# megvii-research/CVPR2023-UniDistill

Measured on AMD Instinct MI355X. Metric: distill-train samples/sec (nuScenes frame); bev_pool+voxelize HBM GB/s, higher is better.
Workload: dtype f32; 1 GPU; camera_exp_distill_lidar: student+teacher distillation step, 6 cams 256x704, 30000-pt cloud, 40 GT boxes, fwd+bwd+AdamW; batch_per_gpu=4, global_batch=4, parallelism=dp1, layout=channels-last dense convs, executor=eager+DDP, strict_no_library_fallthrough=True, wgrad_stream=on, ranks=1, dist_backend=none (single process)

## Files before the change

cvpr2023-unidistill_amd/csrc/conv2d_f32_wino4.hip:

```cpp
#include "ud_common.h"
#include "ud_prof.h"
#include <cstdlib>
#include <type_traits>
#include <utility>
#include <algorithm>

#ifndef UD_W4_ABL
#define UD_W4_ABL 0
#endif

namespace {

typedef float f32x4 __attribute__((ext_vector_type(4)));
typedef float f32x2 __attribute__((ext_vector_type(2)));

constexpr int kT = 32, kTN = 64, kKC = 4, kFQ = 9;
constexpr int kUBytes = kFQ * kTN * kKC * 16;
constexpr int kVBytes = kFQ * kT * kKC * 16;
constexpr int kPBytes = 21504;
constexpr int kP0 = 0, kU0 = 2 * kPBytes, kV0 = kU0 + kUBytes, kV1 = kV0 + kVBytes, kU1 = kV1 + kVBytes;
constexpr int kDump = kU1 + kUBytes;
constexpr int kSmem = kDump + 1024;
constexpr int kStageA = 0, kStageB = kDump - 65536;
static_assert(kStageB >= kV0 && kV1 == kV0 + kVBytes && 65536 <= kV0 + kVBytes, "LDS map");

struct W4Geom {
  int B, H, W, Cin, Cout, bx, by;
  unsigned u_bytes;
  int n_dp, n_units, sk_len;
  float* partial;
};
struct W4Ep {
  const float* bias;
  const float* scale;
  const float* shift;
  const float* residual;
  int relu;
  float* stats;
};

__device__ __forceinline__ void dma16(__amdgpu_buffer_rsrc_t rsrc, unsigned voff, unsigned soff, unsigned lds_wave_base) {
  __builtin_amdgcn_raw_ptr_buffer_load_lds(rsrc, (__attribute__((address_space(3))) void*)(size_t)lds_wave_base, 16, voff, soff, 0, 0);
}
constexpr unsigned kOob = 0xFFF00000u;

__device__ __forceinline__ f32x2 pk_fma(f32x2 a, f32x2 b, f32x2 c) {
  f32x2 d;
  asm("v_pk_fma_f32 %0, %1, %2, %3" : "=v"(d) : "s"(a), "v"(b), "v"(c));
  return d;
}
// ... 75 lines not shown
    u[4] = (1.f / 24.f) * a - (1.f / 12.f) * b + (1.f / 6.f) * cc2;
    u[5] = cc2;
#pragma unroll
    for (int j = 0; j < 6; ++j) {
      const int f = w4_f(r, j);
      out[(f >> 2) * (64 * 16) + (f & 3)] = u[j];
    }
  }
}

template <int N>
struct IC {
  static constexpr int value = N;
};
template <typename F, int... Is>
__device__ __forceinline__ void static_for_impl(F&& f, std::integer_sequence<int, Is...>) {
  (f(IC<Is>{}), ...);
}
template <int N, typename F>
__device__ __forceinline__ void static_for(F&& f) {
  static_for_impl(std::forward<F>(f), std::make_integer_sequence<int, N>{});
}

template <int TWB, int THB>
struct W4Tail {
  const W4Geom& gm;
  const W4Ep& ep;
  int b, ty0, tx0, n0, tid, c4, n;
  float4 bv, scv, shv, s1, s2;
  __device__ W4Tail(const W4Geom& gm_, const W4Ep& ep_, int b_, int ty0_, int tx0_, int n0_, int tid_)
      : gm(gm_), ep(ep_), b(b_), ty0(ty0_), tx0(tx0_), n0(n0_), tid(tid_) {
    c4 = (tid & 15) * 4, n = n0 + c4;
    bv = make_float4(0.f, 0.f, 0.f, 0.f), scv = make_float4(1.f, 1.f, 1.f, 1.f), shv = bv, s1 = bv, s2 = bv;
    if (ep.bias && n < gm.Cout) bv = *reinterpret_cast<const float4*>(ep.bias + n);
    if (ep.scale && n < gm.Cout) {
      scv = *reinterpret_cast<const float4*>(ep.scale + n);
      shv = *reinterpret_cast<const float4*>(ep.shift + n);
    }
  }
  __device__ __forceinline__ void store(float* __restrict__ y, int pass, int row, float4 v) {
    static_assert((TWB & (TWB - 1)) == 0, "tile-block width: a power of two (shift / mask below)");
    const int tl = row >> 4, p = row & 15;
    const int slot = 16 * (tl >> 3) + 4 * ((tl >> 1) & 3) + 2 * pass + (tl & 1);
    const int sy = slot / TWB, sx = slot & (TWB - 1);
    const int gy = 4 * (ty0 + sy) + (p >> 2), gx = 4 * (tx0 + sx) + (p & 3);
    if (slot >= TWB * THB || gy >= gm.H || gx >= gm.W || n >= gm.Cout) return;
    if (ep.bias) { v.x += bv.x; v.y += bv.y; v.z += bv.z; v.w += bv.w; }
    if (ep.scale) {
      v.x = v.x * scv.x + shv.x; v.y = v.y * scv.y + shv.y; v.z = v.z * scv.z + shv.z; v.w = v.w * scv.w + shv.w;
    }
    const size_t off = ((size_t)(b * gm.H + gy) * gm.W + gx) * gm.Cout + n;
    if (ep.residual) {
      const float4 h = *reinterpret_cast<const float4*>(ep.residual + off);
      v.x += h.x; v.y += h.y; v.z += h.z; v.w += h.w;
    }
    if (ep.relu) {
      v.x = fmaxf(v.x, 0.f); v.y = fmaxf(v.y, 0.f); v.z = fmaxf(v.z, 0.f); v.w = fmaxf(v.w, 0.f);
    }
    *reinterpret_cast<float4*>(y + off) = v;
    if (ep.stats) {
      s1.x += v.x; s1.y += v.y; s1.z += v.z; s1.w += v.w;
      s2.x += v.x * v.x; s2.y += v.y * v.y; s2.z += v.z * v.z; s2.w += v.w * v.w;
    }
  }
  __device__ void reduce_stats(float* red, int blk_lin) {
    const int grp = tid >> 4;
    const float a4[4] = {s1.x, s1.y, s1.z, s1.w}, q4[4] = {s2.x, s2.y, s2.z, s2.w};
#pragma unroll
    for (int e = 0; e < 4; ++e) {
      red[(grp * 64 + c4 + e) * 2] = a4[e];
      red[(grp * 64 + c4 + e) * 2 + 1] = q4[e];
    }
    __syncthreads();
    if (tid < 64 && n0 + tid < gm.Cout) {
      double ad = 0.0, qd = 0.0;
      for (int k = 0; k < 32; ++k) {
        ad += (double)red[(k * 64 + tid) * 2];
        qd += (double)red[(k * 64 + tid) * 2 + 1];
      }
      ep.stats[((size_t)blk_lin * gm.Cout + n0 + tid) * 2] = (float)ad;
      ep.stats[((size_t)blk_lin * gm.Cout + n0 + tid) * 2 + 1] = (float)qd;
    }
  }
};

__device__ constexpr int kStepOps[9] = {3, 3, 3, 3, 0, 0, 0, 4, 0};
__host__ __device__ constexpr int w4_wait(int fq) {
  return (fq > 0 ? kStepOps[fq - 1] : 0) + 2 + kStepOps[fq];
}

template <int TWB, int THB>
__global__ __launch_bounds__(512) void k_conv3x3_wino4_f32(const float* __restrict__ x, const float* __restrict__ U,
                                                           float* __restrict__ y, W4Geom gm, W4Ep ep) {
  constexpr int PW = 4 * TWB + 2, PH = 4 * THB + 2;
  constexpr int RP = (TWB == 16) ? PW : (PW | 1);
  constexpr int RB = 2 * RP * 16;
  constexpr int PP = PH * 2 * RP, kPInstr = (PP + 63) / 64;
  static_assert(TWB * THB <= kT && kPInstr * 1024 <= kPBytes && kPInstr <= 24, "tile block");
  constexpr int O0 = 0, O1 = TWB + 1, O2 = 2 * TWB + 2, O3 = 3 * TWB + 2;
  static_assert((O3 + 0) * 4 <= 255 && (O1 + 1) * 4 <= 255, "ds_read2 offsets");
  extern __shared__ __attribute__((aligned(16))) char smem[];
  const unsigned sbase = (unsigned)(size_t)smem;
  const int tid = threadIdx.x, lane = tid & 63;
  const int wave = __builtin_amdgcn_readfirstlane(tid >> 6);
  const int g = lane >> 4, li = lane & 15;
  const int wq = wave & 3, wh = wave >> 2;
  const int nblocks = gm.B * gm.bx * gm.by;
  const int nchunks = gm.Cin / kKC;
  const __amdgpu_buffer_rsrc_t rx = __builtin_amdgcn_make_buffer_rsrc((void*)x, 0, (int)((unsigned)gm.B * gm.H * gm.W * gm.Cin * 4u), 0x00020000);
  const __amdgpu_buffer_rsrc_t ru = __builtin_amdgcn_make_buffer_rsrc((void*)U, 0, (int)gm.u_bytes, 0x00020000);

  int unit, cbi, blk_lin, b, ty0, tx0, n0;
  unsigned po[3];
  unsigned uo;
  unsigned pair_off;
  int nst;
  auto setup = [&](int unit_, int c0, int c1) {
    unit = unit_;
    nst = c1 - c0;
    cbi = unit / nblocks;
    const int ru_ = unit - cbi * nblocks;
    int blk;
    {
      const int base = nblocks >> 3, extra = nblocks & 7, k = ru_ & 7;
      blk = k * base + min(k, extra) + (ru_ >> 3);
    }
    blk_lin = blk;
    b = blk / (gm.bx * gm.by);
    blk -= b * gm.bx * gm.by;
    ty0 = (blk / gm.bx) * THB, tx0 = (blk % gm.bx) * TWB;
    n0 = cbi * kTN;
#pragma unroll
    for (int i = 0; i < 3; ++i) {
      const int pi = wave + 8 * i;
      const int qq = pi * 64 + lane;
      const int qy = qq / (2 * RP), qr = qq - qy * (2 * RP);
      const int qh = qr >= RP ? 1 : 0, qs = qr - qh * RP;
      const int qx = qs < O1 ? 4 * qs : qs < O2 ? 4 * (qs - O1) + 1 : qs < O3 ? 4 * (qs - O2) + 2 : 4 * (qs - O3) + 3;
      const int gy = 4 * ty0 + qy - 1, gx = 4 * tx0 + qx - 1;
      const bool ok = qq < PP && qs < PW && gy >= 0 && gy < gm.H && gx >= 0 && gx < gm.W && !(UD_W4_ABL & (2 | 128));
      po[i] = ok ? (unsigned)(((b * gm.H + gy) * gm.W + gx) * gm.Cin + qh * 4) * 4u : kOob;
    }
    uo = (unsigned)(cbi * nchunks + c0) * (unsigned)kUBytes + wave * 1024;
    pair_off = c0 * 16;
  };
  auto patch_piece = [&](int i, int buf) {
    const int pi = wave + 8 * i;
    dma16(rx, po[i], pair_off, pi < kPInstr ? sbase + kP0 + buf * kPBytes + pi * 1024 : sbase + kDump);
  };
  const unsigned lane16 = lane * 16;
  auto stage_u = [&](int buf) {
    const unsigned ub = sbase + (buf ? kU1 : kU0) + wave * 1024;
#pragma unroll
    for (int i = 0; i < 5; ++i)
      if (i < 4 || wave < 4) dma16(ru, lane16, uo + i * 8192, ub + i * 8192);
  };

  const int grp = wave >> 1;
  const int ttile = (wave & 1) * 16 + (lane & 15), tc = lane >> 4;
  const int ttc = min(ttile, TWB * THB - 1);
  const int tyl = ttc / TWB, txl = ttc - tyl * TWB;
  const unsigned tprow = sbase + kP0 + (4 * tyl) * RB + txl * 16 + tc * 4;
  const int rows4 = grp == 0 ? 0x4420 : grp == 1 ? 0x5531 : 0x1324;
  const unsigned ro1 = (rows4 & 15) * RB, ro2 = ((rows4 >> 4) & 15) * RB, ro3 = ((rows4 >> 8) & 15) * RB, ro4 = ((rows4 >> 12) & 15) * RB;
  const float ca1 = grp < 2 ? 4.f : 1.f, ca2 = grp < 2 ? -5.f : grp == 2 ? -4.f : -1.f;
  const float cb3 = grp == 0 ? 1.f : grp == 1 ? -1.f : grp == 2 ? 1.f : 2.f, cb4 = grp < 2 ? 0.f : grp == 2 ? -4.f : -2.f;
  const unsigned tvbase = sbase + kV0 + (wave & 1) * 1024 + lane * 16;
  const unsigned tdump = sbase + kDump + lane * 16;
  const int q0 = grp < 2 ? 0 : grp == 2 ? 3 : 6;
  const unsigned wA = grp == 1 ? tdump : tvbase + q0 * (kT * kKC * 16);
  const unsigned wB = grp == 1 ? tdump : tvbase + (q0 + 1) * (kT * kKC * 16);
  const unsigned wC = grp == 0 ? tdump : tvbase + (q0 + 1) * (kT * kKC * 16) + 8;
  const unsigned wD = grp == 0 ? tdump : tvbase + (q0 + 2) * (kT * kKC * 16);
  const unsigned vdelta01 = (grp == 1 ? 0 : kVBytes), vdelta23 = (grp == 0 ? 0 : kVBytes);

#define W4_ROWREAD(D, RO)                                                                                               \
  do {                                                                                                                  \
    const unsigned a_ = tprow + (RO);                                                                                   \
    asm volatile("ds_read2_b32 %0, %1 offset0:%2 offset1:%3" : "=v"(D[0]) : "v"(a_), "n"(O0 * 4), "n"(O1 * 4));               \
    asm volatile("ds_read2_b32 %0, %1 offset0:%2 offset1:%3" : "=v"(D[1]) : "v"(a_), "n"(O2 * 4), "n"(O3 * 4));               \
    asm volatile("ds_read2_b32 %0, %1 offset0:%2 offset1:%3" : "=v"(D[2]) : "v"(a_), "n"((O0 + 1) * 4), "n"((O1 + 1) * 4));   \
  } while (0)

  auto row_pass = [](const f32x2 (&w)[3], f32x2 (&v)[3]) {
    const f32x2 c4 = {4.f, 4.f}, c5 = {-5.f, -5.f}, c41 = {-4.f, -1.f}, c12 = {1.f, 2.f}, cn12 = {-1.f, -2.f};
// ... 150 lines not shown
  if (!next_piece()) return;
  setup(p_unit, p_c0, p_c1);
  first_stages();
#pragma unroll 1
  for (;;) {
    asm volatile("s_waitcnt vmcnt(0)" ::: "memory");
    __syncthreads();
    transform_first();
#pragma unroll
    for (int f = 0; f < 36; ++f) acc[f] = (f32x4){0.f, 0.f, 0.f, 0.f};
    asm volatile("s_waitcnt lgkmcnt(0)" ::: "memory");
    __syncthreads();
    asm volatile("ds_read_b128 %0, %1" : "=v"(qa[0]) : "v"(fa));
    asm volatile("ds_read_b128 %0, %1" : "=v"(qb[0]) : "v"(fb0 + kU0));
#pragma unroll 1
    for (int chunk = 0; chunk < nst; chunk += 2) {
      stage(IC<0>{}, chunk);
      stage(IC<1>{}, chunk + 1);
    }
    asm volatile("s_waitcnt vmcnt(0) lgkmcnt(0)" : "+v"(qa[0]), "+v"(qb[0]), "+v"(qa[1]), "+v"(qb[1])::"memory");
    __syncthreads();
    const int e_b = b, e_ty0 = ty0, e_tx0 = tx0, e_n0 = n0, e_blk = blk_lin, e_slot = p_slot;
    const bool more = next_piece();
    W4Tail<TWB, THB> tail(gm, ep, e_b, e_ty0, e_tx0, e_n0, tid);
#pragma unroll
    for (int pass = (UD_W4_ABL & 4) ? 1 : 0; pass < 2; ++pass) {
      float* Os = reinterpret_cast<float*>(smem + (pass ? kStageB : kStageA));
      {
        auto m2 = [&](int i, int j) { return (f32x2){acc[w4_f(i, j)][2 * pass], acc[w4_f(i, j)][2 * pass + 1]}; };
        const f32x2 c2 = {2.f, 2.f}, c4 = {4.f, 4.f}, c8 = {8.f, 8.f};
        f32x2 t[4][6];
#pragma unroll
        for (int j = 0; j < 6; ++j) {
          const f32x2 m1 = m2(1, j), mm2 = m2(2, j), m3 = m2(3, j), m4 = m2(4, j);
          const f32x2 sa = m1 + mm2, da = m1 - mm2, sb = m3 + m4, db = m3 - m4;
          t[0][j] = m2(0, j) + sa + sb;
          t[1][j] = __builtin_elementwise_fma(c2, db, da);
          t[2][j] = __builtin_elementwise_fma(c4, sb, sa);
          t[3][j] = __builtin_elementwise_fma(c8, db, da) + m2(5, j);
        }
        const unsigned o = sbase + (pass ? kStageB : kStageA) + ((wh * 8 + g * 2) * 16 * 64 + (16 * (wq ^ g) + li)) * 4;
#pragma unroll
        for (int a = 0; a < 4; ++a) {
          const f32x2 sa = t[a][1] + t[a][2], da = t[a][1] - t[a][2], sb = t[a][3] + t[a][4], db = t[a][3] - t[a][4];
          const f32x2 y0 = t[a][0] + sa + sb, y1 = __builtin_elementwise_fma(c2, db, da), y2 = __builtin_elementwise_fma(c4, sb, sa),
                      y3 = __builtin_elementwise_fma(c8, db, da) + t[a][5];
          asm volatile("ds_write2st64_b32 %0, %1, %2 offset0:%3 offset1:%4" ::"v"(o), "v"(y0.x), "v"(y0.y), "n"(a * 4 + 0), "n"(a * 4 + 16) : "memory");
// ... 14 lines not shown
#pragma unroll
        for (int k = 0; k < 8; ++k) {
          const int row = (tid >> 4) + 32 * k;
          *reinterpret_cast<float4*>(dst + row * 64 + tail.c4) =
              *reinterpret_cast<const float4*>(Os + row * 64 + (tail.c4 ^ (16 * ((row >> 5) & 3))));
        }
      }
      if (pass == 0) {
        __syncthreads();
        if (more) {
          setup(p_unit, p_c0, p_c1);
          first_stages();
        }
      }
    }
    if (ep.stats && e_slot < 0) {
      __syncthreads();
      tail.reduce_stats(reinterpret_cast<float*>(smem + kStageB), e_blk);
    }
    if (!more) break;
  }
}

template <int TWB, int THB>
__global__ __launch_bounds__(512) void k_wino4_fixup(float* __restrict__ y, W4Geom gm, W4Ep ep) {
  __shared__ float red[32 * 64 * 2];
  const int tid = threadIdx.x;
  const int nblocks = gm.B * gm.bx * gm.by, nchunks = gm.Cin / kKC;
  const int u = gm.n_dp + (blockIdx.x >> 1), pass = blockIdx.x & 1;
  const int base = gm.n_dp * nchunks;
  const int a = u * nchunks - base, e = a + nchunks - 1;
  const int j0 = a / gm.sk_len, j1 = e / gm.sk_len;
  if (j0 == j1) return;
  const int cbi = u / nblocks, ru = u - cbi * nblocks;
  int blk;
  {
    const int bs = nblocks >> 3, extra = nblocks & 7, k = ru & 7;
    blk = k * bs + min(k, extra) + (ru >> 3);
  }
  const int blk_lin = blk;
  const int b = blk / (gm.bx * gm.by);
  blk -= b * gm.bx * gm.by;
  W4Tail<TWB, THB> tail(gm, ep, b, (blk / gm.bx) * THB, (blk % gm.bx) * TWB, cbi * kTN, tid);
  float4 v[8];
#pragma unroll
  for (int k = 0; k < 8; ++k) v[k] = make_float4(0.f, 0.f, 0.f, 0.f);
#pragma unroll 1
  for (int j = j0; j <= j1; ++j) {
    const int first_unit = (base + j * gm.sk_len) / nchunks;
    const int slot = 2 * j + (first_unit == u ? 0 : 1);
    const float* src = gm.partial + ((size_t)slot * 512 + pass * 256 + (tid >> 4)) * 64 + tail.c4;
#pragma unroll
    for (int k = 0; k < 8; ++k) {
      const float4 p = ud_ldg_stream(src + (size_t)k * 32 * 64);
      v[k].x += p.x; v[k].y += p.y; v[k].z += p.z; v[k].w += p.w;
    }
  }
#pragma unroll
  for (int k = 0; k < 8; ++k) tail.store(y, pass, (tid >> 4) + 32 * k, v[k]);
  if (ep.stats) {
    tail.reduce_stats(red, nblocks + 2 * (u - gm.n_dp) + pass);
    if (pass == 0 && tid < 64 && tail.n0 + tid < gm.Cout)
      ep.stats[((size_t)blk_lin * gm.Cout + tail.n0 + tid) * 2] = ep.stats[((size_t)blk_lin * gm.Cout + tail.n0 + tid) * 2 + 1] = 0.f;
  }
}

#undef W4_ROWREAD
#undef W4_COL

struct W4Plan {
  int twb, thb, bx, by;
};
W4Plan w4_plan(int H, int W) {
  static const int shapes[][2] = {{8, 4}, {4, 8}, {16, 2}};
  static const int force = getenv("UD_WINO4_SHAPE") ? atoi(getenv("UD_WINO4_SHAPE")) : -1;
  const int TX = (W + 3) / 4, TY = (H + 3) / 4;
  W4Plan best{};
  long long cost = -1;
  for (int i = 0; i < 3; ++i) {
    if (force >= 0 && i != force) continue;
    const int bx = ud_div_up(TX, shapes[i][0]), by = ud_div_up(TY, shapes[i][1]);
    const long long cst = (long long)bx * by;
    if (cost < 0 || cst < cost) cost = cst, best = W4Plan{shapes[i][0], shapes[i][1], bx, by};
  }
  return best;
}

}

namespace {
std::atomic<int> g_sk_mode{-1};
constexpr int kGrid = 256;
struct W4Sched {
  int grid, n_dp, sk_len;
};
W4Sched w4_schedule(long long units, int nchunks, bool have_ws) {
  static const int env_mode = getenv("UD_WINO4_SK") ? atoi(getenv("UD_WINO4_SK")) : 2;
  const int forced = g_sk_mode.load(std::memory_order_relaxed);
  const int mode = forced >= 0 ? forced : env_mode;
  static const int persist = getenv("UD_WINO4_GRID") ? atoi(getenv("UD_WINO4_GRID")) : kGrid;
  const int G = (int)std::min<long long>(units, persist);
  const int r = (int)(units % G);
  W4Sched sc{G, (int)units, 0};
  if (r == 0 || !have_ws || !mode || (nchunks < 64 && mode < 2)) return sc;
  int len = (int)(((long long)r * nchunks + G - 1) / G);
  len += len & 1;
  if (len + 16 >= (nchunks + 8) * 9 / 10) return sc;
  sc.n_dp = (int)(units - r), sc.sk_len = len;
  return sc;
}
}

extern "C" size_t ud_conv3x3_wino4_f32_weight_bytes(int Cin, int Cout) {
  if (Cin <= 0 || Cout <= 0) return 0;
  return (size_t)ud_div_up(Cout, 64) * ud_div_up(Cin, 4) * kUBytes;
}

extern "C" int ud_conv3x3_wino4_f32_blocks(int H, int W) {
  if (H <= 0 || W <= 0) return 0;
  const W4Plan p = w4_plan(H, W);
  return p.bx * p.by;
}

extern "C" size_t ud_conv3x3_wino4_bnstats_bytes(int B, int H, int W, int Cout) {
  if (B <= 0 || H <= 0 || W <= 0 || Cout <= 0) return 0;
  const W4Plan p = w4_plan(H, W);
  return ((size_t)B * p.bx * p.by + 2 * kGrid) * Cout * 2 * sizeof(float);
}

extern "C" int ud_conv3x3_wino4_f32_weights(const float* w, int64_t s_n, int64_t s_c, int64_t s_y, int64_t s_x, int N, int C,
                                            int flip, float* U, ud_stream_t stream_) {
  if (!w || !U || N <= 0 || C <= 0) return UD_ERR_INVALID_ARG;
  hipStream_t stream = (hipStream_t)stream_;
  UdProfScope prof("conv2d.k_wino4_weights", stream);
  const long long total = (long long)ud_div_up(N, 64) * ud_div_up(C, 4) * 256;
  k_wino4_weights<<<(unsigned)((total + 255) / 256), 256, 0, stream>>>(w, s_n, s_c, s_y, s_x, N, C, flip, U, total);
  UD_LAUNCH_CHECK();
  return UD_OK;
}

extern "C" void ud_conv3x3_wino4_stream_k(int mode) { g_sk_mode.store(mode, std::memory_order_relaxed); }

extern "C" size_t ud_conv3x3_wino4_f32_workspace_bytes(int B, int H, int W, int Cin, int Cout) {
  (void)B; (void)H; (void)W; (void)Cin; (void)Cout;
  return (size_t)2 * kGrid * 512 * 64 * sizeof(float);
}

extern "C" int ud_conv3x3_wino4_nhwc_f32(const float* x, const float* U, float* y, int B, int H, int W, int Cin, int Cout,
                                         const float* bias, const float* scale, const float* shift, const float* residual,
                                         int flags, float* partial, size_t partial_bytes, int* slices, void* workspace,
                                         size_t workspace_bytes, ud_stream_t stream_) {
  if (!x || !U || !y || B <= 0 || H <= 0 || W <= 0 || Cin <= 0 || Cout <= 0) return UD_ERR_INVALID_ARG;
  if ((scale == nullptr) != (shift == nullptr)) return UD_ERR_INVALID_ARG;
  if (Cin % (2 * kKC) != 0 || Cout % 4 != 0) return UD_ERR_UNSUPPORTED;
  hipStream_t stream = (hipStream_t)stream_;
  const W4Plan p = w4_plan(H, W);
  const int nblocks = B * p.bx * p.by;
  const long long units = (long long)nblocks * ud_div_up(Cout, kTN);
  if (units > 0x7fffffffll || (long long)B * H * W * Cin * 4 >= (long long)kOob ||
      ud_conv3x3_wino4_f32_weight_bytes(Cin, Cout) >= (size_t)kOob)
    return UD_ERR_UNSUPPORTED;
  const bool have_ws = workspace && workspace_bytes >= ud_conv3x3_wino4_f32_workspace_bytes(B, H, W, Cin, Cout);
  const W4Sched sc = w4_schedule(units, Cin / kKC, have_ws);
  W4Geom gm{B, H, W, Cin, Cout, p.bx, p.by, (unsigned)ud_conv3x3_wino4_f32_weight_bytes(Cin, Cout), sc.n_dp, (int)units,
            sc.sk_len > 0 ? sc.sk_len : 2, (float*)workspace};
  W4Ep ep{bias, scale, shift, residual, flags & 1, partial};
  if (partial) {
    const size_t rows = (size_t)nblocks + 2 * (size_t)(units - sc.n_dp);
    if (!slices || partial_bytes < rows * Cout * 2 * sizeof(float)) return UD_ERR_WORKSPACE;
    *slices = (int)rows;
    if (rows > (size_t)nblocks)
      ud_zero_f32_async(partial + (size_t)nblocks * Cout * 2, (rows - nblocks) * (size_t)Cout * 2, stream);
  }
  static UdDeviceOnce attr_set;
  if (const unsigned long long attr_set_bit = attr_set.pending()) {
#define UD_W4_ATTR(A, Bq) \
  UD_HIP_TRY(hipFuncSetAttribute((const void*)k_conv3x3_wino4_f32<A, Bq>, hipFuncAttributeMaxDynamicSharedMemorySize, kSmem))
    UD_W4_ATTR(8, 4); UD_W4_ATTR(4, 8); UD_W4_ATTR(16, 2);
#undef UD_W4_ATTR
    attr_set.mark(attr_set_bit);
  }
  UdProfScope prof("conv2d.k_conv3x3_wino4_f32", stream);
  const dim3 grid((unsigned)sc.grid);
  const int n_sk = (int)units - sc.n_dp;
#define UD_W4_LAUNCH(A, Bq)                                                                    \
  do {                                                                                         \
    k_conv3x3_wino4_f32<A, Bq><<<grid, 512, kSmem, stream>>>(x, U, y, gm, ep);                 \
    if (n_sk > 0) k_wino4_fixup<A, Bq><<<2 * n_sk, 512, 0, stream>>>(y, gm, ep);               \
  } while (0)
  if (p.twb == 8) UD_W4_LAUNCH(8, 4);
  else if (p.twb == 4) UD_W4_LAUNCH(4, 8);
  else UD_W4_LAUNCH(16, 2);
#undef UD_W4_LAUNCH
  UD_LAUNCH_CHECK();
  return UD_OK;
}
```

cvpr2023-unidistill_amd/unidistill_amd/_lib.py:

```python
import ctypes
import os

import torch

_HERE = os.path.dirname(os.path.abspath(__file__))
LIB_PATH = os.path.join(_HERE, "_lib", "libunidistill_hip.so")
_cdll = None

c_void_p, c_int, c_size_t, c_uint, c_i64, c_float = (
    ctypes.c_void_p, ctypes.c_int, ctypes.c_size_t, ctypes.c_uint, ctypes.c_int64, ctypes.c_float)

_SIGS = {
    "ud_version": (ctypes.c_char_p, []),
    "ud_abi_version": (c_int, []),
    "ud_error_string": (ctypes.c_char_p, [c_int]),
    "ud_prof_enable": (None, [c_int]),
    "ud_prof_read": (c_int, [ctypes.c_char_p, ctypes.POINTER(ctypes.c_double), ctypes.POINTER(c_int), c_int]),
    "ud_bench_stream": (c_int, [c_void_p, c_void_p, c_size_t, c_int, c_void_p]),
    "ud_bev_pool_workspace_bytes": (c_size_t, [c_int] * 6),
    "ud_bev_pool_fwd": (c_int, [c_void_p] * 4 + [c_int] * 6 + [c_uint, c_void_p, c_size_t, c_void_p]),
    "ud_bev_pool_bwd_workspace_bytes": (c_size_t, [c_int] * 4 + [c_i64]),
    "ud_bev_pool_bwd": (c_int, [c_void_p] + [c_i64] * 4 + [c_void_p, c_void_p] + [c_int] * 5
                        + [c_void_p, c_size_t, c_void_p]),
    "ud_lss_prepare_mats": (c_int, [c_void_p] * 6 + [c_int, c_int, c_void_p, c_void_p]),
# ... 95 lines not shown
                            + [c_size_t, c_void_p]),
    "ud_lidar_prep_compact": (c_int, [c_void_p, c_i64, c_int, c_void_p, c_void_p, c_int, c_int] + [c_void_p] * 6
                              + [c_i64, c_int, c_void_p, c_i64, c_void_p, c_size_t, c_void_p]),
    "ud_jpeg_parse": (c_int, [c_void_p, c_i64, c_void_p]),
    "ud_jpeg_plan": (c_size_t, [c_void_p, c_int]),
    "ud_jpeg_decode": (c_int, [c_void_p, c_i64, c_void_p, c_void_p, c_int, c_void_p, c_i64, c_void_p, c_void_p,
                               c_void_p, c_size_t, c_void_p]),
    "ud_nus_pred_to_global": (c_int, [c_void_p, c_i64, c_int] + [c_void_p] * 3 + [c_int, c_void_p, c_int]
                              + [c_void_p] * 7),
    "ud_nus_eval_workspace_bytes": (c_size_t, [c_i64, c_int]),
    "ud_nus_eval": (c_int, [c_void_p, c_void_p, c_int, c_i64, c_void_p, c_size_t, c_void_p]),
    "ud_stem_pack_weights": (c_int, [c_void_p] + [c_i64] * 4 + [c_void_p]),
    "ud_stem_conv7x7_bn_relu": (c_int, [c_void_p] + [c_i64] * 4 + [c_int] * 3 + [c_void_p] * 4 + [c_int, c_void_p]),
    "ud_maxpool3x3s2_nhwc": (c_int, [c_void_p] * 2 + [c_int] * 5 + [c_void_p]),
    "ud_conv1x1_wgrad_workspace_bytes": (c_size_t, [c_i64, c_int, c_int]),
    "ud_conv3x3_wgrad_f32_workspace_bytes": (c_size_t, [c_int] * 5),
    "ud_conv3x3_wgrad_nhwc_f32": (c_int, [c_void_p] * 3 + [c_int] * 5 + [c_void_p, c_size_t, c_void_p]),
    "ud_conv1x1_wgrad_f32_workspace_bytes": (c_size_t, [c_i64, c_int, c_int]),
    "ud_conv1x1_wgrad_mapped_nhwc_f32": (c_int, [c_void_p] * 3 + [c_i64, c_int, c_int] + [c_void_p] * 2
                                         + [c_void_p, c_size_t, c_void_p]),
    "ud_conv3x3_wino4_f32_weight_bytes": (c_size_t, [c_int, c_int]),
    "ud_conv3x3_wino4_bnstats_bytes": (c_size_t, [c_int] * 4),
    "ud_conv3x3_wino4_f32_blocks": (c_int, [c_int, c_int]),
    "ud_conv3x3_wino4_f32_weights": (c_int, [c_void_p] + [c_i64] * 4 + [c_int] * 3 + [c_void_p, c_void_p]),
    "ud_conv3x3_wino4_f32_workspace_bytes": (c_size_t, [c_int] * 5),
    "ud_conv3x3_wino4_stream_k": (None, [c_int]),
    "ud_conv3x3_wino4_nhwc_f32": (c_int, [c_void_p] * 3 + [c_int] * 5 + [c_void_p] * 4 + [c_int, c_void_p, c_size_t,
                                                                                              c_void_p, c_void_p, c_size_t, c_void_p]),
    "ud_conv3x3_wino_f32_weight_bytes": (c_size_t, [c_int, c_int]),
    "ud_conv3x3_wino_bnstats_bytes": (c_size_t, [c_int] * 4),
    "ud_conv3x3_wino4_wgrad_f32_workspace_bytes": (c_size_t, [c_int] * 5),
    "ud_conv3x3_wino4_wgrad_nhwc_f32": (c_int, [c_void_p] * 3 + [c_int] * 5 + [c_void_p, c_size_t, c_void_p]),
    "ud_conv3x3_wino_wgrad_f32_workspace_bytes": (c_size_t, [c_int] * 5),
    "ud_conv3x3_wino_wgrad_nhwc_f32": (c_int, [c_void_p] * 3 + [c_int] * 5 + [c_void_p, c_size_t, c_void_p]),
    "ud_conv3x3_wino_f32_blocks": (c_int, [c_int, c_int]),
    "ud_conv3x3_wino_f32_weights": (c_int, [c_void_p] + [c_i64] * 4 + [c_int] * 3 + [c_void_p, c_void_p]),
    "ud_conv3x3_wino_nhwc_f32": (c_int, [c_void_p] * 3 + [c_int] * 5 + [c_void_p] * 4 + [c_int, c_void_p, c_size_t,
                                                                                        c_void_p, c_void_p]),
    "ud_conv1x1_wgrad_nhwc_bf16": (c_int, [c_void_p] * 3 + [c_i64, c_int, c_int] + [c_void_p, c_size_t, c_void_p]),
    "ud_assign_targets": (c_int, [c_void_p] + [c_int] * 3 + [c_void_p, c_void_p] + [c_int] * 8 + [c_float] * 5
                          + [c_void_p] * 6),
    "ud_det_loss_workspace_bytes": (c_size_t, [c_int]),
    "ud_det_focal_fwd": (c_int, [c_void_p] * 3 + [c_int] * 4 + [c_void_p, c_float, c_float, c_void_p, c_void_p,
                                                                c_void_p, c_size_t, c_void_p]),
    "ud_det_focal_bwd": (c_int, [c_void_p] + [c_int] * 4 + [c_void_p] * 5 + [c_float, c_float, c_void_p,
                                                                              c_void_p]),
# ... 173 lines not shown
```

cvpr2023-unidistill_amd/unidistill_amd/ops/conv2d_f32.py:

```python
import ctypes
import os

import torch

from .. import _lib
from . import bn_act, wgrad_stream


def _nhwc(t):
    return t if t.is_contiguous(memory_format=torch.channels_last) else \
        t.contiguous(memory_format=torch.channels_last)


def supported(x, weight, ks):
    return (x.is_cuda and x.dtype == torch.float32 and x.dim() == 4 and weight.dtype == torch.float32
            and tuple(weight.shape[2:]) == (ks, ks) and weight.shape[1] % 32 == 0 and weight.shape[0] % 4 == 0
            and x.shape[1] == weight.shape[1])


def _bn_partial(nbytes, dev):
    return torch.empty(max(int(nbytes) // 4, 1), dtype=torch.float32, device=dev), ctypes.c_int(0)


FLOP_COUNTER = None
SHAPE_LOG = None


USE_WINOGRAD = os.environ.get("UD_F32_WINOGRAD", "1") != "0"
WINO_MIN_FILL = 0.7
USE_WINOGRAD_WGRAD = os.environ.get("UD_F32_WINOGRAD_WGRAD", "1") != "0"


USE_WINO4 = os.environ.get("UD_F32_WINO4", "1") != "0"
WINO4_MIN_FILL = float(os.environ.get("UD_F32_WINO4_FILL", "0.35"))


WINO4_MIN_CIN = int(os.environ.get("UD_F32_WINO4_CIN", "256"))


def wino4_pays(H, W, cin, cout):
    if not (USE_WINOGRAD and USE_WINO4) or cin % 8 or cout % 4:
        return False
    blocks = _lib.load().ud_conv3x3_wino4_f32_blocks(H, W)
    fill = WINO4_MIN_FILL if (cin <= 1024 or WINO4_MIN_FILL == 0.0) else max(WINO4_MIN_FILL, 0.7)
    if ((H + 3) // 4) * ((W + 3) // 4) < fill * 32 * blocks:
        return False
    return WINO4_MIN_FILL == 0.0 or cin >= WINO4_MIN_CIN or H * W >= 128 * 128


USE_WINO4_WGRAD = os.environ.get("UD_F32_WINO4_WGRAD", "1") != "0"
WINO4_WGRAD_ALL = False


def wino4_wgrad_pays(B, H, W, cin, cout):
    if not (USE_WINO4 and USE_WINO4_WGRAD) or cin % 32 or cout % 64 or B * H * W * max(cin, cout) * 4 >= 2 ** 31 - 1:
        return False
    return WINO4_WGRAD_ALL or (wino4_pays(H, W, cin, cout) and H * W >= 11000)


def wino_pays(H, W, cin, cout):
    if not USE_WINOGRAD or cin % 8 or cout % 4:
        return False
    blocks = _lib.load().ud_conv3x3_wino_f32_blocks(H, W)
    return ((H + 1) // 2) * ((W + 1) // 2) >= WINO_MIN_FILL * 64 * blocks


def _wino_weights(weight, transposed, f4=False):
    lib = _lib.load()
# ... 14 lines not shown
            weight._ud_wino = None
        return make()
    key = (bool(transposed), bool(f4), weight._version, weight.data_ptr(), tuple(weight.shape), tuple(weight.stride()))
    cache = getattr(weight, "_ud_wino", None)
    if cache is not None and cache[0] == key:
        return cache[1]
    U = make()
    try:
        weight._ud_wino = (key, U)
    except (AttributeError, RuntimeError):
        pass
    return U


def _launch3(x, weight, bias=None, relu=False, transposed=False, bn_stats=False, scale=None, shift=None):
    B, cin, H, W = x.shape
    cout = weight.shape[1] if transposed else weight.shape[0]
    if FLOP_COUNTER is not None:
        FLOP_COUNTER[0] += 2 * B * H * W * cout * 9 * cin
    if SHAPE_LOG is not None:
        SHAPE_LOG.append((B, cin, H, W, cout, bool(transposed)))
    lib = _lib.load()
    y = torch.empty((B, cout, H, W), dtype=torch.float32, device=x.device, memory_format=torch.channels_last)
    if wino4_pays(H, W, cin, cout):
        U = _wino_weights(weight, transposed, f4=True)
        part, ns = (None, ctypes.c_int(0))
        if bn_stats:
            part, ns = _bn_partial(lib.ud_conv3x3_wino4_bnstats_bytes(B, H, W, cout), x.device)
        ws = _lib.workspace(x.device, lib.ud_conv3x3_wino4_f32_workspace_bytes(B, H, W, cin, cout), "conv_w4")
        _lib.check(lib.ud_conv3x3_wino4_nhwc_f32(_lib.ptr(x), _lib.ptr(U), _lib.ptr(y), B, H, W, cin, cout, _lib.ptr(bias),
                                                 _lib.ptr(scale), _lib.ptr(shift), None, 1 if relu else 0, _lib.ptr(part),
                                                 part.numel() * 4 if bn_stats else 0, ctypes.addressof(ns), _lib.ptr(ws),
                                                 ws.numel(), _lib.stream_of(x)),
                   "ud_conv3x3_wino4_nhwc_f32")
        return (y, (part, ns.value, B * H * W)) if bn_stats else y
    if wino_pays(H, W, cin, cout):
        U = _wino_weights(weight, transposed)
        part, ns = (None, ctypes.c_int(0))
        if bn_stats:
            part, ns = _bn_partial(lib.ud_conv3x3_wino_bnstats_bytes(B, H, W, cout), x.device)
        _lib.check(lib.ud_conv3x3_wino_nhwc_f32(_lib.ptr(x), _lib.ptr(U), _lib.ptr(y), B, H, W, cin, cout, _lib.ptr(bias),
                                                _lib.ptr(scale), _lib.ptr(shift), None, 1 if relu else 0, _lib.ptr(part), part.numel() * 4 if bn_stats else 0,
                                                ctypes.addressof(ns), _lib.stream_of(x)), "ud_conv3x3_wino_nhwc_f32")
        return (y, (part, ns.value, B * H * W)) if bn_stats else y
    w = weight.detach()
    w_tap = (w.permute(1, 2, 3, 0) if transposed else w.permute(0, 2, 3, 1)).contiguous()
    if bn_stats:
# ... 208 lines not shown
```

include/unidistill_hip.h:

```cpp
#ifndef UNIDISTILL_HIP_H
#define UNIDISTILL_HIP_H

#include <stddef.h>
#include <stdint.h>

#ifdef __cplusplus
extern "C" {
#endif

typedef void* ud_stream_t;

#define UD_OK 0
#define UD_ERR_INVALID_ARG (-1)
#define UD_ERR_WORKSPACE (-2)
#define UD_ERR_HIP (-3)
#define UD_ERR_UNSUPPORTED (-4)

const char* ud_version(void);
int ud_abi_version(void);
const char* ud_error_string(int code);

void ud_prof_enable(int on);
int ud_prof_read(const char* name, double* total_ms, int* calls, int reset);

// ... 253 lines not shown
int ud_conv1x1_wgrad_mapped_nhwc_bf16(const void* x, const void* dy, float* dw, int64_t P, int Cin, int Cout,
                                      const int* x_map, const int* dy_map, void* workspace,
                                      size_t workspace_bytes, ud_stream_t stream);
size_t ud_conv3x3_wgrad_f32_workspace_bytes(int B, int H, int W, int Cin, int Cout);
int ud_conv3x3_wgrad_nhwc_f32(const float* x, const float* dy, float* dw, int B, int H, int W, int Cin, int Cout,
                              void* workspace, size_t workspace_bytes, ud_stream_t stream);
size_t ud_conv1x1_wgrad_f32_workspace_bytes(int64_t P, int Cin, int Cout);
int ud_conv1x1_wgrad_mapped_nhwc_f32(const float* x, const float* dy, float* dw, int64_t P, int Cin, int Cout,
                                     const int* x_map, const int* dy_map, void* workspace, size_t workspace_bytes,
                                     ud_stream_t stream);

size_t ud_conv3x3_wino_f32_weight_bytes(int Cin, int Cout);
size_t ud_conv3x3_wino_bnstats_bytes(int B, int H, int W, int Cout);
int ud_conv3x3_wino_f32_blocks(int H, int W);
int ud_conv3x3_wino_f32_weights(const float* w, int64_t s_n, int64_t s_c, int64_t s_y, int64_t s_x, int N, int C, int flip,
                                float* U, ud_stream_t stream);
int ud_conv3x3_wino_nhwc_f32(const float* x, const float* U, float* y, int B, int H, int W, int Cin, int Cout,
                             const float* bias, const float* scale, const float* shift, const float* residual, int flags,
                             float* partial, size_t partial_bytes, int* slices, ud_stream_t stream);

size_t ud_conv3x3_wino4_f32_weight_bytes(int Cin, int Cout);
size_t ud_conv3x3_wino4_bnstats_bytes(int B, int H, int W, int Cout);
int ud_conv3x3_wino4_f32_blocks(int H, int W);
int ud_conv3x3_wino4_f32_weights(const float* w, int64_t s_n, int64_t s_c, int64_t s_y, int64_t s_x, int N, int C, int flip,
                                 float* U, ud_stream_t stream);
size_t ud_conv3x3_wino4_f32_workspace_bytes(int B, int H, int W, int Cin, int Cout);
void ud_conv3x3_wino4_stream_k(int mode);
int ud_conv3x3_wino4_nhwc_f32(const float* x, const float* U, float* y, int B, int H, int W, int Cin, int Cout,
                              const float* bias, const float* scale, const float* shift, const float* residual, int flags,
                              float* partial, size_t partial_bytes, int* slices, void* workspace, size_t workspace_bytes,
                              ud_stream_t stream);

size_t ud_conv3x3_wino_wgrad_f32_workspace_bytes(int B, int H, int W, int Cin, int Cout);
int ud_conv3x3_wino_wgrad_nhwc_f32(const float* x, const float* dy, float* dw, int B, int H, int W, int Cin, int Cout,
                                   void* workspace, size_t workspace_bytes, ud_stream_t stream);

size_t ud_conv3x3_wino4_wgrad_f32_workspace_bytes(int B, int H, int W, int Cin, int Cout);
int ud_conv3x3_wino4_wgrad_nhwc_f32(const float* x, const float* dy, float* dw, int B, int H, int W, int Cin, int Cout,
                                    void* workspace, size_t workspace_bytes, ud_stream_t stream);

int ud_points_transform(const float* in, float* out, const int64_t* seg, const double* mats, const float* last,
                        int S, int D, int64_t max_rows, ud_stream_t stream);

int ud_image_normalize(const unsigned char* img, float* out, const float* mean, const float* std, int to_rgb,
                       int NI, int H, int W, int out_channels_last, ud_stream_t stream);
int ud_collate_pad(const float* const* samples, const int64_t* rows, int B, int64_t L, int W, float* out,
// ... 230 lines not shown
```

Baseline: 68.95 samples/s.

## Pack tiles from multiple batch images into one Winograd F(4,3) tile block

```diff
diff --git a/cvpr2023-unidistill_amd/csrc/conv2d_f32_wino4.hip b/cvpr2023-unidistill_amd/csrc/conv2d_f32_wino4.hip
--- a/cvpr2023-unidistill_amd/csrc/conv2d_f32_wino4.hip
+++ b/cvpr2023-unidistill_amd/csrc/conv2d_f32_wino4.hip
@@ -17,15 +17,18 @@
 constexpr int kT = 32, kTN = 64, kKC = 4, kFQ = 9;
 constexpr int kUBytes = kFQ * kTN * kKC * 16;
 constexpr int kVBytes = kFQ * kT * kKC * 16;
-constexpr int kPBytes = 21504;
+constexpr int kPBytes = 22528;
 constexpr int kP0 = 0, kU0 = 2 * kPBytes, kV0 = kU0 + kUBytes, kV1 = kV0 + kVBytes, kU1 = kV1 + kVBytes;
 constexpr int kDump = kU1 + kUBytes;
 constexpr int kSmem = kDump + 1024;
 constexpr int kStageA = 0, kStageB = kDump - 65536;
-static_assert(kStageB >= kV0 && kV1 == kV0 + kVBytes && 65536 <= kV0 + kVBytes, "LDS map");
+static_assert(kP0 == 0 && kU0 == 45056 && kV0 == 81920 && kV1 == 100352 && kU1 == 118784 && kDump == 155648 && kSmem == 156672 &&
+                  kSmem <= 163840 && kStageB >= kV0 && kV1 == kV0 + kVBytes && 65536 <= kV0 + kVBytes,
+              "LDS map");
 
 struct W4Geom {
   int B, H, W, Cin, Cout, bx, by;
+  int nblocks;
   unsigned u_bytes;
   int n_dp, n_units, sk_len;
   float* partial;
@@ -147,7 +150,7 @@
   static_for_impl(std::forward<F>(f), std::make_integer_sequence<int, N>{});
 }
 
-template <int TWB, int THB>
+template <int TWB, int THB, int TB>
 struct W4Tail {
   const W4Geom& gm;
   const W4Ep& ep;
@@ -167,14 +170,16 @@
     static_assert((TWB & (TWB - 1)) == 0, "tile-block width: a power of two (shift / mask below)");
     const int tl = row >> 4, p = row & 15;
     const int slot = 16 * (tl >> 3) + 4 * ((tl >> 1) & 3) + 2 * pass + (tl & 1);
-    const int sy = slot / TWB, sx = slot & (TWB - 1);
+    const int si = TB > 1 ? slot / (TWB * THB) : 0, sl = slot - si * (TWB * THB);
+    const int sy = sl / TWB, sx = sl & (TWB - 1);
+    const int bi = b + si;
     const int gy = 4 * (ty0 + sy) + (p >> 2), gx = 4 * (tx0 + sx) + (p & 3);
-    if (slot >= TWB * THB || gy >= gm.H || gx >= gm.W || n >= gm.Cout) return;
+    if (slot >= TWB * THB * TB || (TB > 1 && bi >= gm.B) || gy >= gm.H || gx >= gm.W || n >= gm.Cout) return;
     if (ep.bias) { v.x += bv.x; v.y += bv.y; v.z += bv.z; v.w += bv.w; }
     if (ep.scale) {
       v.x = v.x * scv.x + shv.x; v.y = v.y * scv.y + shv.y; v.z = v.z * scv.z + shv.z; v.w = v.w * scv.w + shv.w;
     }
-    const size_t off = ((size_t)(b * gm.H + gy) * gm.W + gx) * gm.Cout + n;
+    const size_t off = ((size_t)(bi * gm.H + gy) * gm.W + gx) * gm.Cout + n;
     if (ep.residual) {
       const float4 h = *reinterpret_cast<const float4*>(ep.residual + off);
       v.x += h.x; v.y += h.y; v.z += h.z; v.w += h.w;
@@ -214,14 +219,15 @@
   return (fq > 0 ? kStepOps[fq - 1] : 0) + 2 + kStepOps[fq];
 }
 
-template <int TWB, int THB>
+template <int TWB, int THB, int TB>
 __global__ __launch_bounds__(512) void k_conv3x3_wino4_f32(const float* __restrict__ x, const float* __restrict__ U,
                                                            float* __restrict__ y, W4Geom gm, W4Ep ep) {
   constexpr int PW = 4 * TWB + 2, PH = 4 * THB + 2;
   constexpr int RP = (TWB == 16) ? PW : (PW | 1);
   constexpr int RB = 2 * RP * 16;
-  constexpr int PP = PH * 2 * RP, kPInstr = (PP + 63) / 64;
-  static_assert(TWB * THB <= kT && kPInstr * 1024 <= kPBytes && kPInstr <= 24, "tile block");
+  constexpr int PPS = PH * 2 * RP;
+  constexpr int PP = TB * PPS, kPInstr = (PP + 63) / 64;
+  static_assert(TWB * THB * TB <= kT && kPInstr * 1024 <= kPBytes && kPInstr <= 24, "tile block");
   constexpr int O0 = 0, O1 = TWB + 1, O2 = 2 * TWB + 2, O3 = 3 * TWB + 2;
   static_assert((O3 + 0) * 4 <= 255 && (O1 + 1) * 4 <= 255, "ds_read2 offsets");
   extern __shared__ __attribute__((aligned(16))) char smem[];
@@ -230,7 +236,7 @@
   const int wave = __builtin_amdgcn_readfirstlane(tid >> 6);
   const int g = lane >> 4, li = lane & 15;
   const int wq = wave & 3, wh = wave >> 2;
-  const int nblocks = gm.B * gm.bx * gm.by;
+  const int nblocks = gm.nblocks;
   const int nchunks = gm.Cin / kKC;
   const __amdgpu_buffer_rsrc_t rx = __builtin_amdgcn_make_buffer_rsrc((void*)x, 0, (int)((unsigned)gm.B * gm.H * gm.W * gm.Cin * 4u), 0x00020000);
   const __amdgpu_buffer_rsrc_t ru = __builtin_amdgcn_make_buffer_rsrc((void*)U, 0, (int)gm.u_bytes, 0x00020000);
@@ -253,18 +259,20 @@
     blk_lin = blk;
     b = blk / (gm.bx * gm.by);
     blk -= b * gm.bx * gm.by;
+    b *= TB;
     ty0 = (blk / gm.bx) * THB, tx0 = (blk % gm.bx) * TWB;
     n0 = cbi * kTN;
 #pragma unroll
     for (int i = 0; i < 3; ++i) {
       const int pi = wave + 8 * i;
       const int qq = pi * 64 + lane;
-      const int qy = qq / (2 * RP), qr = qq - qy * (2 * RP);
+      const int qi = TB > 1 ? qq / PPS : 0, qp = qq - qi * PPS;
+      const int qy = qp / (2 * RP), qr = qp - qy * (2 * RP);
       const int qh = qr >= RP ? 1 : 0, qs = qr - qh * RP;
       const int qx = qs < O1 ? 4 * qs : qs < O2 ? 4 * (qs - O1) + 1 : qs < O3 ? 4 * (qs - O2) + 2 : 4 * (qs - O3) + 3;
       const int gy = 4 * ty0 + qy - 1, gx = 4 * tx0 + qx - 1;
-      const bool ok = qq < PP && qs < PW && gy >= 0 && gy < gm.H && gx >= 0 && gx < gm.W && !(UD_W4_ABL & (2 | 128));
-      po[i] = ok ? (unsigned)(((b * gm.H + gy) * gm.W + gx) * gm.Cin + qh * 4) * 4u : kOob;
+      const bool ok = qq < PP && (TB == 1 || b + qi < gm.B) && qs < PW && gy >= 0 && gy < gm.H && gx >= 0 && gx < gm.W && !(UD_W4_ABL & (2 | 128));
+      po[i] = ok ? (unsigned)((((b + qi) * gm.H + gy) * gm.W + gx) * gm.Cin + qh * 4) * 4u : kOob;
     }
     uo = (unsigned)(cbi * nchunks + c0) * (unsigned)kUBytes + wave * 1024;
     pair_off = c0 * 16;
@@ -283,9 +291,10 @@
 
   const int grp = wave >> 1;
   const int ttile = (wave & 1) * 16 + (lane & 15), tc = lane >> 4;
-  const int ttc = min(ttile, TWB * THB - 1);
-  const int tyl = ttc / TWB, txl = ttc - tyl * TWB;
-  const unsigned tprow = sbase + kP0 + (4 * tyl) * RB + txl * 16 + tc * 4;
+  const int ttc = min(ttile, TWB * THB * TB - 1);
+  const int tim = ttc / (TWB * THB), ttl = ttc - tim * (TWB * THB);
+  const int tyl = ttl / TWB, txl = ttl - tyl * TWB;
+  const unsigned tprow = sbase + kP0 + tim * (PPS * 16) + (4 * tyl) * RB + txl * 16 + tc * 4;
   const int rows4 = grp == 0 ? 0x4420 : grp == 1 ? 0x5531 : 0x1324;
   const unsigned ro1 = (rows4 & 15) * RB, ro2 = ((rows4 >> 4) & 15) * RB, ro3 = ((rows4 >> 8) & 15) * RB, ro4 = ((rows4 >> 12) & 15) * RB;
   const float ca1 = grp < 2 ? 4.f : 1.f, ca2 = grp < 2 ? -5.f : grp == 2 ? -4.f : -1.f;
@@ -482,7 +491,7 @@
     __syncthreads();
     const int e_b = b, e_ty0 = ty0, e_tx0 = tx0, e_n0 = n0, e_blk = blk_lin, e_slot = p_slot;
     const bool more = next_piece();
-    W4Tail<TWB, THB> tail(gm, ep, e_b, e_ty0, e_tx0, e_n0, tid);
+    W4Tail<TWB, THB, TB> tail(gm, ep, e_b, e_ty0, e_tx0, e_n0, tid);
 #pragma unroll
     for (int pass = (UD_W4_ABL & 4) ? 1 : 0; pass < 2; ++pass) {
       float* Os = reinterpret_cast<float*>(smem + (pass ? kStageB : kStageA));
@@ -543,11 +552,11 @@
   }
 }
 
-template <int TWB, int THB>
+template <int TWB, int THB, int TB>
 __global__ __launch_bounds__(512) void k_wino4_fixup(float* __restrict__ y, W4Geom gm, W4Ep ep) {
   __shared__ float red[32 * 64 * 2];
   const int tid = threadIdx.x;
-  const int nblocks = gm.B * gm.bx * gm.by, nchunks = gm.Cin / kKC;
+  const int nblocks = gm.nblocks, nchunks = gm.Cin / kKC;
   const int u = gm.n_dp + (blockIdx.x >> 1), pass = blockIdx.x & 1;
   const int base = gm.n_dp * nchunks;
   const int a = u * nchunks - base, e = a + nchunks - 1;
@@ -562,7 +571,7 @@
   const int blk_lin = blk;
   const int b = blk / (gm.bx * gm.by);
   blk -= b * gm.bx * gm.by;
-  W4Tail<TWB, THB> tail(gm, ep, b, (blk / gm.bx) * THB, (blk % gm.bx) * TWB, cbi * kTN, tid);
+  W4Tail<TWB, THB, TB> tail(gm, ep, b * TB, (blk / gm.bx) * THB, (blk % gm.bx) * TWB, cbi * kTN, tid);
   float4 v[8];
 #pragma unroll
   for (int k = 0; k < 8; ++k) v[k] = make_float4(0.f, 0.f, 0.f, 0.f);
@@ -590,19 +599,23 @@
 #undef W4_COL
 
 struct W4Plan {
-  int twb, thb, bx, by;
+  int shape, tb, bx, by;
+  long long nblocks;
 };
-W4Plan w4_plan(int H, int W) {
-  static const int shapes[][2] = {{8, 4}, {4, 8}, {16, 2}};
+constexpr int kShapes[][3] = {{8, 4, 1}, {4, 8, 1}, {16, 2, 1}, {4, 4, 2}, {8, 2, 2}};
+constexpr int kNShapes = 5, kNShapes1 = 3;
+W4Plan w4_plan(int B, int H, int W) {
   static const int force = getenv("UD_WINO4_SHAPE") ? atoi(getenv("UD_WINO4_SHAPE")) : -1;
+  static const int pack = getenv("UD_WINO4_PACK") ? atoi(getenv("UD_WINO4_PACK")) : 1;
   const int TX = (W + 3) / 4, TY = (H + 3) / 4;
   W4Plan best{};
   long long cost = -1;
-  for (int i = 0; i < 3; ++i) {
-    if (force >= 0 && i != force) continue;
-    const int bx = ud_div_up(TX, shapes[i][0]), by = ud_div_up(TY, shapes[i][1]);
-    const long long cst = (long long)bx * by;
-    if (cost < 0 || cst < cost) cost = cst, best = W4Plan{shapes[i][0], shapes[i][1], bx, by};
+  for (int i = 0; i < (pack ? kNShapes : kNShapes1); ++i) {
+    if (force >= 0 && force < kNShapes && i != force) continue;
+    if (i == kNShapes1 && force < 0 && cost >= 0 && (long long)B * TX * TY * 4 >= cost * kT * 3) break;
+    const int bx = ud_div_up(TX, kShapes[i][0]), by = ud_div_up(TY, kShapes[i][1]);
+    const long long cst = (long long)ud_div_up(B, kShapes[i][2]) * bx * by;
+    if (cost < 0 || cst < cost) cost = cst, best = W4Plan{i, kShapes[i][2], bx, by, cst};
   }
   return best;
 }
@@ -623,6 +636,14 @@
   const int G = (int)std::min<long long>(units, persist);
   const int r = (int)(units % G);
   W4Sched sc{G, (int)units, 0};
+  static const int short_grid = getenv("UD_WINO4_SHORT") ? atoi(getenv("UD_WINO4_SHORT")) : 16;
+  if (units < persist && persist <= kGrid && short_grid && have_ws && mode && !(nchunks < 64 && mode < 2)) {
+    int len = (int)((units * nchunks + persist - 1) / persist);
+    len = std::max(len, short_grid);
+    len += len & 1;
+    if (len + 16 >= (nchunks + 8) * 9 / 10) return sc;
+    return W4Sched{(int)((units * nchunks + len - 1) / len), 0, len};
+  }
   if (r == 0 || !have_ws || !mode || (nchunks < 64 && mode < 2)) return sc;
   int len = (int)(((long long)r * nchunks + G - 1) / G);
   len += len & 1;
@@ -639,14 +660,20 @@
 
 extern "C" int ud_conv3x3_wino4_f32_blocks(int H, int W) {
   if (H <= 0 || W <= 0) return 0;
-  const W4Plan p = w4_plan(H, W);
+  const W4Plan p = w4_plan(1, H, W);
   return p.bx * p.by;
+}
+
+extern "C" int ud_conv3x3_wino4_f32_slots(int B, int H, int W) {
+  if (B <= 0 || H <= 0 || W <= 0) return 0;
+  const W4Plan p = w4_plan(B, H, W);
+  return p.nblocks * kT > 0x7fffffffll ? 0x7fffffff : (int)(p.nblocks * kT);
 }
 
 extern "C" size_t ud_conv3x3_wino4_bnstats_bytes(int B, int H, int W, int Cout) {
   if (B <= 0 || H <= 0 || W <= 0 || Cout <= 0) return 0;
-  const W4Plan p = w4_plan(H, W);
-  return ((size_t)B * p.bx * p.by + 2 * kGrid) * Cout * 2 * sizeof(float);
+  const W4Plan p = w4_plan(B, H, W);
+  return ((size_t)p.nblocks + 2 * kGrid) * Cout * 2 * sizeof(float);
 }
 
 extern "C" int ud_conv3x3_wino4_f32_weights(const float* w, int64_t s_n, int64_t s_c, int64_t s_y, int64_t s_x, int N, int C,
@@ -675,15 +702,17 @@
   if ((scale == nullptr) != (shift == nullptr)) return UD_ERR_INVALID_ARG;
   if (Cin % (2 * kKC) != 0 || Cout % 4 != 0) return UD_ERR_UNSUPPORTED;
   hipStream_t stream = (hipStream_t)stream_;
-  const W4Plan p = w4_plan(H, W);
-  const int nblocks = B * p.bx * p.by;
-  const long long units = (long long)nblocks * ud_div_up(Cout, kTN);
+  const W4Plan p = w4_plan(B, H, W);
+  const long long units = p.nblocks * ud_div_up(Cout, kTN);
+  const int nblocks = (int)p.nblocks;
   if (units > 0x7fffffffll || (long long)B * H * W * Cin * 4 >= (long long)kOob ||
       ud_conv3x3_wino4_f32_weight_bytes(Cin, Cout) >= (size_t)kOob)
     return UD_ERR_UNSUPPORTED;
   const bool have_ws = workspace && workspace_bytes >= ud_conv3x3_wino4_f32_workspace_bytes(B, H, W, Cin, Cout);
   const W4Sched sc = w4_schedule(units, Cin / kKC, have_ws);
-  W4Geom gm{B, H, W, Cin, Cout, p.bx, p.by, (unsigned)ud_conv3x3_wino4_f32_weight_bytes(Cin, Cout), sc.n_dp, (int)units,
+  if ((units - sc.n_dp) >= kGrid || (sc.sk_len > 0 && (size_t)2 * sc.grid * 512 * 64 * sizeof(float) > workspace_bytes))
+    return UD_ERR_WORKSPACE;
+  W4Geom gm{B, H, W, Cin, Cout, p.bx, p.by, nblocks, (unsigned)ud_conv3x3_wino4_f32_weight_bytes(Cin, Cout), sc.n_dp, (int)units,
             sc.sk_len > 0 ? sc.sk_len : 2, (float*)workspace};
   W4Ep ep{bias, scale, shift, residual, flags & 1, partial};
   if (partial) {
@@ -695,23 +724,27 @@
   }
   static UdDeviceOnce attr_set;
   if (const unsigned long long attr_set_bit = attr_set.pending()) {
-#define UD_W4_ATTR(A, Bq) \
-  UD_HIP_TRY(hipFuncSetAttribute((const void*)k_conv3x3_wino4_f32<A, Bq>, hipFuncAttributeMaxDynamicSharedMemorySize, kSmem))
-    UD_W4_ATTR(8, 4); UD_W4_ATTR(4, 8); UD_W4_ATTR(16, 2);
+#define UD_W4_ATTR(A, Bq, T) \
+  UD_HIP_TRY(hipFuncSetAttribute((const void*)k_conv3x3_wino4_f32<A, Bq, T>, hipFuncAttributeMaxDynamicSharedMemorySize, kSmem))
+    UD_W4_ATTR(8, 4, 1); UD_W4_ATTR(4, 8, 1); UD_W4_ATTR(16, 2, 1); UD_W4_ATTR(4, 4, 2); UD_W4_ATTR(8, 2, 2);
 #undef UD_W4_ATTR
     attr_set.mark(attr_set_bit);
   }
   UdProfScope prof("conv2d.k_conv3x3_wino4_f32", stream);
   const dim3 grid((unsigned)sc.grid);
   const int n_sk = (int)units - sc.n_dp;
-#define UD_W4_LAUNCH(A, Bq)                                                                    \
+#define UD_W4_LAUNCH(A, Bq, T)                                                                 \
   do {                                                                                         \
-    k_conv3x3_wino4_f32<A, Bq><<<grid, 512, kSmem, stream>>>(x, U, y, gm, ep);                 \
-    if (n_sk > 0) k_wino4_fixup<A, Bq><<<2 * n_sk, 512, 0, stream>>>(y, gm, ep);               \
+    k_conv3x3_wino4_f32<A, Bq, T><<<grid, 512, kSmem, stream>>>(x, U, y, gm, ep);              \
+    if (n_sk > 0) k_wino4_fixup<A, Bq, T><<<2 * n_sk, 512, 0, stream>>>(y, gm, ep);            \
   } while (0)
-  if (p.twb == 8) UD_W4_LAUNCH(8, 4);
-  else if (p.twb == 4) UD_W4_LAUNCH(4, 8);
-  else UD_W4_LAUNCH(16, 2);
+  switch (p.shape) {
+    case 0: UD_W4_LAUNCH(8, 4, 1); break;
+    case 1: UD_W4_LAUNCH(4, 8, 1); break;
+    case 2: UD_W4_LAUNCH(16, 2, 1); break;
+    case 3: UD_W4_LAUNCH(4, 4, 2); break;
+    default: UD_W4_LAUNCH(8, 2, 2); break;
+  }
 #undef UD_W4_LAUNCH
   UD_LAUNCH_CHECK();
   return UD_OK;
diff --git a/cvpr2023-unidistill_amd/unidistill_amd/_lib.py b/cvpr2023-unidistill_amd/unidistill_amd/_lib.py
--- a/cvpr2023-unidistill_amd/unidistill_amd/_lib.py
+++ b/cvpr2023-unidistill_amd/unidistill_amd/_lib.py
@@ -141,6 +141,7 @@
     "ud_conv3x3_wino4_f32_weight_bytes": (c_size_t, [c_int, c_int]),
     "ud_conv3x3_wino4_bnstats_bytes": (c_size_t, [c_int] * 4),
     "ud_conv3x3_wino4_f32_blocks": (c_int, [c_int, c_int]),
+    "ud_conv3x3_wino4_f32_slots": (c_int, [c_int] * 3),
     "ud_conv3x3_wino4_f32_weights": (c_int, [c_void_p] + [c_i64] * 4 + [c_int] * 3 + [c_void_p, c_void_p]),
     "ud_conv3x3_wino4_f32_workspace_bytes": (c_size_t, [c_int] * 5),
     "ud_conv3x3_wino4_stream_k": (None, [c_int]),
diff --git a/cvpr2023-unidistill_amd/unidistill_amd/ops/conv2d_f32.py b/cvpr2023-unidistill_amd/unidistill_amd/ops/conv2d_f32.py
--- a/cvpr2023-unidistill_amd/unidistill_amd/ops/conv2d_f32.py
+++ b/cvpr2023-unidistill_amd/unidistill_amd/ops/conv2d_f32.py
@@ -38,12 +38,15 @@
 WINO4_MIN_CIN = int(os.environ.get("UD_F32_WINO4_CIN", "256"))
 
 
-def wino4_pays(H, W, cin, cout):
+def wino4_pays(H, W, cin, cout, B=None):
     if not (USE_WINOGRAD and USE_WINO4) or cin % 8 or cout % 4:
         return False
-    blocks = _lib.load().ud_conv3x3_wino4_f32_blocks(H, W)
+    if B is None:
+        B, slots = 1, 32 * _lib.load().ud_conv3x3_wino4_f32_blocks(H, W)
+    else:
+        slots = _lib.load().ud_conv3x3_wino4_f32_slots(B, H, W)
     fill = WINO4_MIN_FILL if (cin <= 1024 or WINO4_MIN_FILL == 0.0) else max(WINO4_MIN_FILL, 0.7)
-    if ((H + 3) // 4) * ((W + 3) // 4) < fill * 32 * blocks:
+    if B * ((H + 3) // 4) * ((W + 3) // 4) < fill * slots:
         return False
     return WINO4_MIN_FILL == 0.0 or cin >= WINO4_MIN_CIN or H * W >= 128 * 128
 
@@ -104,7 +107,7 @@
         SHAPE_LOG.append((B, cin, H, W, cout, bool(transposed)))
     lib = _lib.load()
     y = torch.empty((B, cout, H, W), dtype=torch.float32, device=x.device, memory_format=torch.channels_last)
-    if wino4_pays(H, W, cin, cout):
+    if wino4_pays(H, W, cin, cout, B):
         U = _wino_weights(weight, transposed, f4=True)
         part, ns = (None, ctypes.c_int(0))
         if bn_stats:
diff --git a/include/unidistill_hip.h b/include/unidistill_hip.h
--- a/include/unidistill_hip.h
+++ b/include/unidistill_hip.h
@@ -299,6 +299,7 @@
 size_t ud_conv3x3_wino4_f32_weight_bytes(int Cin, int Cout);
 size_t ud_conv3x3_wino4_bnstats_bytes(int B, int H, int W, int Cout);
 int ud_conv3x3_wino4_f32_blocks(int H, int W);
+int ud_conv3x3_wino4_f32_slots(int B, int H, int W);
 int ud_conv3x3_wino4_f32_weights(const float* w, int64_t s_n, int64_t s_c, int64_t s_y, int64_t s_x, int N, int C, int flip,
                                  float* U, ud_stream_t stream);
 size_t ud_conv3x3_wino4_f32_workspace_bytes(int B, int H, int W, int Cin, int Cout);
```

Result: no change. 68.81 samples/s (-0.2%).
